# zijieli-Jlee/Temporal-Pointcloud-Upsampling-GAN

Measured on AMD Instinct MI355X. Metric: GAN train-steps/sec (G+D) on 4096-pt x3-frame clips, higher is better.
Workload: dtype bf16; 1 GPU; cfg2: 4096-pt x3-frame fluid clips, full G+D adversarial step (SRNet(3,128) + FluidTempoDis(3) + FluidSpatialDis, Adam), all-keep mask regime, gate open, even iteration; batch 8 per GPU; per_gpu_batch=8, global_batch=8, parallelism=dp1, step_mode=hipgraph (1 graph per step)

## Files before the change

### include/tpgan_ops.h

```cpp
#ifndef TPGAN_OPS_H
#define TPGAN_OPS_H

#include <stddef.h>
#include <stdint.h>

#ifdef __cplusplus
extern "C" {
#endif

typedef enum {
    TPG_OK = 0,
    TPG_ERR_ARG = -1,
    TPG_ERR_LAUNCH = -2,
    TPG_ERR_UNSUPPORTED = -3
} tpg_status;

#define TPG_MAX_K 64

const char *tpg_version(void);
const char *tpg_target_arch(void);

int tpg_knn_f32(const float *p1, const float *p2, const int64_t *len1,
                const int64_t *len2, int B, int P1, int P2, int D, int K,
                float r2, float *dist, int64_t *idx, void *stream);

int tpg_knn_grid_f32(const float *p1, const float *p2, const int64_t *len1, const int64_t *len2, int B,
                     int P1, int P2, int K, float *dist, int64_t *idx, void *ws, void *stream);

int tpg_knn_mfma_f32(const float *p1, const float *p2, const int64_t *len1,
                     const int64_t *len2, int B, int P1, int P2, int D, int K,
                     float *dist, int64_t *idx, int redo, void *stream);

int tpg_knn_small_f32(const float *p1, const float *p2, const int64_t *len1,
                      const int64_t *len2, int B, int P1, int P2, int D, int K,
                      float *dist, int64_t *idx, int redo, void *stream);

size_t tpg_frnn_grid_workspace_bytes(int B, int P2);
int tpg_frnn_grid_f32(const float *p1, const float *p2, const int64_t *len1, const int64_t *len2, int B, int P1,
                      int P2, int K, float r, float *dist, int64_t *idx, void *ws, void *stream);

int tpg_chamfer_fwd_f32(const float *src, const float *tgt, int B, int N, int M,
                        float *d1, int64_t *i1, float *d2, int64_t *i2,
                        void *stream);
size_t tpg_chamfer_bwd_workspace_bytes(int B, int N, int M);
int tpg_chamfer_bwd_f32(const float *src, const float *tgt, int B, int N, int M,
                        const int64_t *i1, const int64_t *i2, const float *g1,
                        const float *g2, float *gsrc, float *gtgt, void *ws, void *stream);

int tpg_fps_f32(const float *xyz, int B, int N, int m, float *temp, int32_t *idx,
                void *stream);

int tpg_fps_prefix_f32(const float *xyz, int B, int N, int m, float *temp, int32_t *idx,
                       const int32_t *prefix_in, int32_t *prefix_out, void *stream);

int tpg_fps_start_f32(const float *xyz, const int32_t *start, int skip_origin, int B, int N, int m,
                      float *temp, int32_t *idx, void *stream);

int tpg_gather_fwd_f32(const float *feat, const int32_t *idx, int B, int C, int N,
                       int S, float *out, void *stream);
int tpg_gather_bwd_f32(const float *gout, const int32_t *idx, int B, int C, int N,
                       int S, float *gfeat, void *stream);

int tpg_gather_rows_fwd_f32(const float *rows, const int32_t *idx, int B, int N, int S, int C, float *out, void *stream);
int tpg_gather_rows_bwd_f32(const float *gout, const int32_t *idx, int B, int N, int S, int C, float *grows,
                            void *stream);

int tpg_ball_query_f32(const float *xyz, const float *new_xyz, int B, int N, int S,
                       float radius, int nsample, int32_t *idx, void *stream);

int tpg_group_fwd_f32(const float *feat, const int32_t *idx, int B, int C, int N,
                      int S, int K, float *out, void *stream);
int tpg_group_bwd_f32(const float *gout, const int32_t *idx, int B, int C, int N,
                      int S, int K, float *gfeat, void *stream);

int tpg_three_nn_f32(const float *unknown, const float *known, int B, int n, int m,
                     float *dist2, int32_t *idx, void *stream);
int tpg_three_interp_fwd_f32(const float *feat, const int32_t *idx, const float *w,
                             int B, int C, int m, int n, float *out, void *stream);
int tpg_three_interp_bwd_f32(const float *gout, const int32_t *idx, const float *w,
                             int B, int C, int m, int n, float *gfeat,
                             void *stream);

typedef enum { TPG_DTYPE_F32 = 0, TPG_DTYPE_BF16 = 1 } tpg_dtype;

int tpg_rowcombine_fwd(const void *U, const void *QE, const int32_t *idx, int mode, int dtype_in,
                       int dtype_out, int B, int N, int S, int K, int C, float slope, void *out,
                       void *stream);

int tpg_invert_index(const int32_t *idx, int B, int N, int SK, int32_t *offs, int32_t *list,
                     int32_t *tmp, void *stream);

int tpg_rowcombine_bwd(const void *gout, const int32_t *idx, const int32_t *offs, const int32_t *list,
                       const void *E, int mode, int dtype_in, int dtype_out, int B, int N, int S, int K,
                       int C, float slope, void *gU, void *gQE, void *stream);

int tpg_rowcombine_edge_fwd(const void *Y, const int32_t *idx, int dtype_in, int dtype_out, int B, int N, int K, int C,
                            float slope_a, float slope_e, void *out, void *stream);
int tpg_rowcombine_edge_bwd(const void *gout, const int32_t *idx, const int32_t *offs, const int32_t *list,
                            const void *Y, int dtype_in, int dtype_out, int B, int N, int K, int C, float slope_a,
                            float slope_e, void *gY, void *stream);

int tpg_head_bn_act_fwd(const float *h, int B, int C, const float *gamma, const float *beta, float *running_mean,
                        float *running_var, long long *num_batches_tracked, float momentum, float eps, float slope,
                        const float *mask, float *y, float *mean, float *rstd, void *stream);
int tpg_head_bn_act_bwd(const float *gy, const float *h, const float *mean, const float *rstd, const float *gamma,
                        const float *beta, float slope, const float *mask, int B, int C, float *dh, float *dgamma,
                        float *dbeta, void *stream);

#define TPG_BN_PHASE_ALL 0
#define TPG_BN_PHASE_STATS 1
#define TPG_BN_PHASE_APPLY 2
size_t tpg_rowbn_workspace_bytes(int C, int nseg);
int tpg_rowbn_fwd(const void *x, int dtype_in, long long P, int K, int C, float eps, float momentum,
                  int training, float *running_mean, float *running_var, long long *num_batches_tracked,
                  const float *mean_shift, const float *gamma, const float *beta, float slope, float *mean,
                  float *rstd, void *y,
                  int dtype_out, uint8_t *argmax, void *ws, int nseg, int phase, void *stream);
int tpg_rowbn_bwd(const void *gy, int dtype_g, const void *x, int dtype_in, const uint8_t *argmax,
                  const void *y, int dtype_y, long long P, int K, int C, int training, const float *mean,
                  const float *rstd, const float *gamma, const float *beta, float slope, float *dgamma,
                  float *dbeta, void *dx, void *ws, int nseg, int phase, void *stream);

int tpg_rowbn_bwd_sums(const void *gy, int dtype_g, const void *x, int dtype_in, const uint8_t *argmax,
                       const void *y, int dtype_y, long long P, int K, int C, int training, const float *mean,
                       const float *rstd, const float *gamma, const float *beta, float slope, float *dgamma,
                       float *dbeta, float *c12, void *ws, int nseg, void *stream);

int tpg_rowbn_stats_consts(const void *x, int dtype_in, long long P, int C, float eps, float momentum,
                           float *running_mean, float *running_var, long long *num_batches_tracked,
                           const float *mean_shift, const float *gamma, const float *beta, float *mean, float *rstd,
                           float *ci, void *ws, int nseg, void *stream);
int tpg_rowbn_bwd_sums_consts(const void *gy, int dtype_g, const void *x, int dtype_in, const uint8_t *argmax,
                              const void *y, int dtype_y, long long P, int K, int C, int training, const float *mean,
                              const float *rstd, const float *gamma, const float *beta, float slope, float *dgamma,
                              float *dbeta, float *c12, float *cb, void *ag, void *ws, int nseg, void *stream);

size_t tpg_mlp_workspace_bytes(int C, int nseg);
int tpg_mlp_fwd(const void *x, long long P, int Cin, int Cout, int nseg, const float *ss_in, int ss_stride,
                float slope_in, const float *W, int w_per_seg, void *y, float eps, float momentum,
                float *running_mean, float *running_var, long long *num_batches_tracked, const float *mean_shift,
                const float *gamma_out, const float *beta_out, float *mean_out, float *rstd_out, float *ci_out,
                void *ws, void *stream);

int tpg_mlp_consts(const float *mean, const float *rstd, const float *gamma, const float *beta, const float *c12,
                   int C, int nseg, float *ci, float *cb, void *stream);
int tpg_mlp_max_prep(const void *gout, const void *y, const float *cb_out, float slope_out, long long rows, int C,
                     int nseg, void *ag, void *stream);
int tpg_mlp_dgrad(const void *x_out, const void *g_out, const uint8_t *arg, int K, const float *cb_out,
                  const void *x_in, const float *ci_in, float slope_in, const float *W,
                  int w_per_seg, long long P, int Cin, int Cout, int nseg, int mode, void *g_in, float *c12_in,
                  float *dgamma_in, float *dbeta_in, float *cb_in, void *ws, void *stream);
size_t tpg_mlp_wgrad_workspace_bytes(long long P, int Cin, int Cout, int nseg);
int tpg_mlp_wgrad(const void *x_out, const void *g_out, const uint8_t *arg, int K, const float *cb_out,
                  const void *x_in, const float *ci_in, float slope_in, long long P, int Cin,
                  int Cout, int nseg, int mode, float *dW, void *ws, void *stream);
int tpg_mlp_bn_bwd_apply(const void *g, const void *x, const float *ci, const float *c12, long long P, int C,
                         int nseg, void *dx, void *stream);
int tpg_mlp_bn_bwd_apply_rowsum(const void *g, const void *x, const float *ci, const float *c12, long long P, int K,
                                int C, int nseg, void *dx, float *qneg, void *stream);

int tpg_mlp_infer_supported(int C0, int C1, int C2, int K);
int tpg_mlp_infer_fwd(const void *U, const void *Q, const int32_t *idx, int dtype_in, int B, int N, int S, int K, int C0,
                      int C1, int C2, const void *W1p, const void *W2p, const float *a1, const float *c1, const float *a2,
                      const float *c2, float slope0, float slope1, float slope2, void *out, void *stream);

int tpg_spectral_norm_fwd(const float *W, float *u, float *v, int R, int Cn, int iterate, float eps,
                          float *Wsn, float *sigma, void *stream);
int tpg_spectral_norm_bwd(const float *G, const float *Wsn, const float *u, const float *v,
                          const float *sigma, int R, int Cn, float *dW, void *stream);

long long tpg_spectral_norm_multi_stride(int R, int Cn);
int tpg_spectral_norm_multi_fwd(const void *desc, int M, int max_rc, float *out, int iterate, float eps,
                                void *stream);
// ... 129 lines not shown
```

### temporal-pointcloud-upsampling-gan_amd/_lib.py

```python
import ctypes as C
import os

_HERE = os.path.dirname(os.path.abspath(__file__))
LIB_PATH = os.environ.get("TPGAN_HIP_LIBRARY") or os.path.join(_HERE, "csrc", "libtpgan_hip.so")

_P = C.c_void_p
_I = C.c_int
_F = C.c_float
_L = C.c_longlong

SIGNATURES = {
    "tpg_knn_f32": [_P, _P, _P, _P, _I, _I, _I, _I, _I, _F, _P, _P, _P],
    "tpg_knn_mfma_f32": [_P, _P, _P, _P, _I, _I, _I, _I, _I, _P, _P, _I, _P],
    "tpg_knn_small_f32": [_P, _P, _P, _P, _I, _I, _I, _I, _I, _P, _P, _I, _P],
    "tpg_knn_grid_f32": [_P, _P, _P, _P, _I, _I, _I, _I, _P, _P, _P, _P],
    "tpg_frnn_grid_f32": [_P, _P, _P, _P, _I, _I, _I, _I, _F, _P, _P, _P, _P],
    "tpg_chamfer_fwd_f32": [_P, _P, _I, _I, _I, _P, _P, _P, _P, _P],
    "tpg_chamfer_bwd_f32": [_P, _P, _I, _I, _I, _P, _P, _P, _P, _P, _P, _P, _P],
    "tpg_fps_f32": [_P, _I, _I, _I, _P, _P, _P],
    "tpg_fps_prefix_f32": [_P, _I, _I, _I, _P, _P, _P, _P, _P],
    "tpg_fps_start_f32": [_P, _P, _I, _I, _I, _I, _P, _P, _P],
    "tpg_gather_fwd_f32": [_P, _P, _I, _I, _I, _I, _P, _P],
    "tpg_gather_bwd_f32": [_P, _P, _I, _I, _I, _I, _P, _P],
    "tpg_ball_query_f32": [_P, _P, _I, _I, _I, _F, _I, _P, _P],
    "tpg_group_fwd_f32": [_P, _P, _I, _I, _I, _I, _I, _P, _P],
    "tpg_group_bwd_f32": [_P, _P, _I, _I, _I, _I, _I, _P, _P],
    "tpg_three_nn_f32": [_P, _P, _I, _I, _I, _P, _P, _P],
    "tpg_three_interp_fwd_f32": [_P, _P, _P, _I, _I, _I, _I, _P, _P],
    "tpg_three_interp_bwd_f32": [_P, _P, _P, _I, _I, _I, _I, _P, _P],
    "tpg_gather_rows_fwd_f32": [_P, _P, _I, _I, _I, _I, _P, _P],
    "tpg_gather_rows_bwd_f32": [_P, _P, _I, _I, _I, _I, _P, _P],
    "tpg_rowcombine_fwd": [_P, _P, _P, _I, _I, _I, _I, _I, _I, _I, _I, _F, _P, _P],
    "tpg_invert_index": [_P, _I, _I, _I, _P, _P, _P, _P],
    "tpg_rowcombine_bwd": [_P, _P, _P, _P, _P, _I, _I, _I, _I, _I, _I, _I, _I, _F, _P, _P, _P],
    "tpg_rowcombine_edge_fwd": [_P, _P, _I, _I, _I, _I, _I, _I, _F, _F, _P, _P],
    "tpg_rowcombine_edge_bwd": [_P, _P, _P, _P, _P, _I, _I, _I, _I, _I, _I, _F, _F, _P, _P],
    "tpg_head_bn_act_fwd": [_P, _I, _I, _P, _P, _P, _P, _P, _F, _F, _F, _P, _P, _P, _P, _P],
    "tpg_head_bn_act_bwd": [_P, _P, _P, _P, _P, _P, _F, _P, _I, _I, _P, _P, _P, _P],
    "tpg_rowbn_fwd": [_P, _I, _L, _I, _I, _F, _F, _I, _P, _P, _P, _P, _P, _P, _F, _P, _P, _P, _I, _P, _P, _I, _I, _P],
    "tpg_rowbn_bwd": [_P, _I, _P, _I, _P, _P, _I, _L, _I, _I, _I, _P, _P, _P, _P, _F, _P, _P, _P, _P, _I, _I, _P],
    "tpg_cubic_interp_f32": [_P, _P, _P, _I, _I, _I, _I, _F, _P, _P, _P, _P],
    "tpg_spectral_norm_fwd": [_P, _P, _P, _I, _I, _I, _F, _P, _P, _P],
    "tpg_spectral_norm_bwd": [_P, _P, _P, _P, _P, _I, _I, _P, _P],
    "tpg_spectral_norm_multi_fwd": [_P, _I, _I, _P, _I, _F, _P],
    "tpg_spectral_norm_multi_fwd_split": [_P, _P, _I, _I, _P, _P, _L, _F, _P],
    "tpg_spectral_norm_multi_bwd": [_P, _I, _I, _P, _P, _P, _P, _P],
    "tpg_rowbn_bwd_sums": [_P, _I, _P, _I, _P, _P, _I, _L, _I, _I, _I, _P, _P, _P, _P, _F, _P, _P, _P, _P, _I, _P],
    "tpg_rowbn_bwd_sums_consts": [_P, _I, _P, _I, _P, _P, _I, _L, _I, _I, _I, _P, _P, _P, _P, _F, _P, _P, _P, _P, _P, _P, _I, _P],
    "tpg_rowbn_stats_consts": [_P, _I, _L, _I, _F, _F, _P, _P, _P, _P, _P, _P, _P, _P, _P, _P, _I, _P],
    "tpg_mlp_consts": [_P, _P, _P, _P, _P, _I, _I, _P, _P, _P],
    "tpg_mlp_max_prep": [_P, _P, _P, _F, _L, _I, _I, _P, _P],
    "tpg_mlp_dgrad": [_P, _P, _P, _I, _P, _P, _P, _F, _P, _I, _L, _I, _I, _I, _I, _P, _P, _P, _P, _P, _P, _P],
    "tpg_mlp_wgrad": [_P, _P, _P, _I, _P, _P, _P, _F, _L, _I, _I, _I, _I, _P, _P, _P],
    "tpg_mlp_bn_bwd_apply": [_P, _P, _P, _P, _L, _I, _I, _P, _P],
    "tpg_mlp_bn_bwd_apply_rowsum": [_P, _P, _P, _P, _L, _I, _I, _I, _P, _P, _P],
    "tpg_small_tail_fwd": [_P, _I, _P, _P, _F, _F, _L, _I, _I, _I, _I, _P, _P, _P],
    "tpg_small_tail_bwd": [_P, _P, _P, _P, _I, _P, _P, _F, _F, _L, _I, _I, _I, _I, _P, _P, _P, _P, _P],
    "tpg_rowlinear_fwd": [_P, _I, _P, _P, _L, _I, _I, _I, _F, _P, _I, _P],
    "tpg_rowlinear_dgrad": [_P, _P, _I, _P, _L, _I, _I, _I, _F, _P, _I, _P],
    "tpg_rowlinear_wgrad": [_P, _I, _P, _P, _I, _L, _I, _I, _I, _F, _P, _P, _P, _P],
    "tpg_mlp_fwd": [_P, _L, _I, _I, _I, _P, _I, _F, _P, _I, _P, _F, _F, _P, _P, _P, _P, _P, _P, _P, _P, _P, _P, _P],
    "tpg_mlp_infer_fwd": [_P, _P, _P, _I, _I, _I, _I, _I, _I, _I, _I, _P, _P, _P, _P, _P, _P, _F, _F, _F, _P, _P],
    "tpg_context_expand_f32": [_P, _P, _P, _I, _I, _I, _I, _P, _P, _P, _P, _P],
    "tpg_radius_reduce_f32": [_P, _P, _P, _P, _I, _I, _I, _F, _I, _P, _P, _P, _P],
    "tpg_radius_reduce_exhaustive_f32": [_P, _P, _P, _P, _I, _I, _I, _F, _I, _P, _P, _P],
    "tpg_patch_select_f32": [_P, _L, _P, _P, _P, _I, _I, _P, _P, _P],
    "tpg_clip_gather_high_f32": [_P, _P, _L, _P, _P, _P, _I, _P, _P, _I, _I, _I, _P, _P, _P],
    "tpg_clip_gather_low_f32": [_P, _P, _P, _F, _P, _L, _P, _P, _I, _I, _I, _I, _P, _P, _P],
    "tpg_frame_subset": [_P, _P, _I, _I, _P, _P],
    "tpg_action_gather_f32": [_P, _L, _P, _P, _P, _P, _I, _I, _I, _I, _P, _P, _P],
    "tpg_replace_dummy_centres": [_P, _P, _P, _I, _I, _I, _I, _P, _P, _P, _P],
    "tpg_emd_init_f32": [_P, _I, _I, _I, _I, _P, _P, _P],
    "tpg_emd_rounds_f32": [_P, _I, _I, _F, _F, _I, _I, _I, _I, _I, _P, _P, _P],
    "tpg_emd_finish_f32": [_P, _I, _I, _P, _P, _P, _P, _P, _P],
    "tpg_gaussian_row_sums_f32": [_P, _P, _P, _P, _I, _I, _I, _F, _P, _P],
    "tpg_render_points_f32": [_P, _P, _P, _I, _I, _P, _I, _I, _I, _I, _F, _F, _P, _P, _P, _P, _P, _P],
    "tpg_render_spheres_f32": [_P, _P, _I, _I, _P, _I, _I, _I, _F, _P, _P, _P, _P],
    "tpg_surface_smooth_f32": [_P, _I, _I, _I, _I, _F, _P, _P],
    "tpg_surface_shade_f32": [_P, _P, _P, _I, _I, _P, _I, _I, _I, _F, _F, _P, _P, _P, _P, _P],
    "tpg_pbf_predict_f32": [_P, _P, _P, _P, _I, _I, _F, _F, _P, _P, _P, _P],
    "tpg_pbf_grid_f32": [_P, _P, _I, _I, _F, _P, _P],
    "tpg_pbf_lambda_f32": [_P, _P, _I, _I, _F, _F, _F, _P, _P, _P, _P],
    "tpg_pbf_dp_f32": [_P, _P, _P, _P, _I, _I, _F, _F, _F, _F, _F, _P, _P, _P, _P],
    "tpg_pbf_finish_f32": [_P, _P, _P, _I, _I, _F, _F, _F, _P, _P, _P, _P],
    "tpg_iso_count_f32": [_P, _I, _I, _I, _F, _P, _P, _P],
    "tpg_iso_emit_f32": [_P, _I, _I, _I, _P, _F, _F, _P, _L, _L, _P, _P, _P, _P],
    "tpg_aniso_kernels_f32": [_P, _P, _I, _I, _F, _F, _F, _F, _F, _F, _F, _I, _I, _P, _P, _P, _P, _P, _P],
    "tpg_aniso_kernels_exhaustive_f32": [_P, _P, _I, _I, _F, _F, _F, _F, _F, _F, _F, _I, _I, _P, _P, _P, _P, _P, _P],
    "tpg_aniso_field_f32": [_P, _P, _P, _P, _P, _P, _I, _I, _I, _F, _F, _P, _P, _P],
    "tpg_aniso_field_exhaustive_f32": [_P, _P, _P, _P, _P, _P, _I, _I, _I, _F, _F, _P, _P],
}
SIZE_GETTERS = ("tpg_rowbn_workspace_bytes", "tpg_mlp_workspace_bytes", "tpg_context_expand_workspace_bytes",
                "tpg_emd_workspace_bytes", "tpg_pbf_workspace_bytes", "tpg_iso_workspace_bytes",
                "tpg_aniso_workspace_bytes")
OTHER_GETTERS = ("tpg_spectral_norm_multi_stride", "tpg_spectral_norm_multi_bwd_scratch",
                 "tpg_mlp_wgrad_workspace_bytes", "tpg_frnn_grid_workspace_bytes", "tpg_small_tail_workspace_bytes",
                 "tpg_chamfer_bwd_workspace_bytes", "tpg_rowlinear_wgrad_workspace_bytes", "tpg_rowlinear_supported",
                 "tpg_spectral_norm_split_rows", "tpg_spectral_norm_split_max_cn", "tpg_spectral_norm_split_max_rows",
                 "tpg_patch_select_workspace_bytes", "tpg_patch_select_max_k", "tpg_mlp_infer_supported")
STRING_GETTERS = ("tpg_version", "tpg_target_arch")

STATUS = {0: "TPG_OK", -1: "TPG_ERR_ARG", -2: "TPG_ERR_LAUNCH", -3: "TPG_ERR_UNSUPPORTED"}

_lib = None


class HipLibraryMissing(RuntimeError):
    pass


def load():
    global _lib
    if _lib is not None:
        return _lib
    if not os.path.exists(LIB_PATH):
        raise HipLibraryMissing(
# ... 45 lines not shown
```

### temporal-pointcloud-upsampling-gan_amd/csrc/invert_index.hpp

```cpp
#pragma once
#include "tpg_common.hpp"

namespace tpg_inv {

constexpr int kWaves = 16;
constexpr int kThreads = kWaves * 64;
constexpr int kMaxBins = 256;
constexpr int kHist = kMaxBins * kWaves;
constexpr int kUnroll = 8;
constexpr int kMaxLdsBytes = 160 * 1024;
constexpr int kFixedInts = 2 * kHist + 64;
constexpr int kMaxCntRows = kMaxLdsBytes / 4 - kFixedInts;

struct Plan {
    int bits, passes, ebits, pack, use_cnt;
    size_t smem;
};

inline int ceil_log2(long long v) {
    int b = 0;
    while ((1LL << b) < v) ++b;
    return b;
}

// ... 109 lines not shown
    }

    for (int p = 0; p < passes; ++p) {
        volatile int *cur = hist0 + (p & 1) * kHist, *nxt = hist0 + ((p + 1) & 1) * kHist;
        const bool last = p + 1 == passes;
        const int32_t *src = p == 0 ? nullptr : (((passes - p) & 1) ? tp : ls);
        int32_t *dst = ((passes - 1 - p) & 1) ? tp : ls;
        const bool packed_in = src != nullptr && pack;
        block_exclusive_scan(cur, L, wsum, tid);
        if (!last) {
            for (int i = tid; i < L; i += kThreads) nxt[i] = 0;
            __syncthreads();
        }
        const int dshift = p ? (p - 1) * bits : 0;
        int raw[kUnroll], rawn[kUnroll];
#pragma unroll
        for (int u = 0; u < kUnroll; ++u) {
            const int i = e_lo + u * 64 + lane;
            raw[u] = i < e_hi ? (src ? src[i] : i) : 0;
        }
        for (int base = e_lo; base < e_hi; base += 64 * kUnroll) {
            int ev[kUnroll], dg[kUnroll], kh[kUnroll];
#pragma unroll
            for (int u = 0; u < kUnroll; ++u) {
                const int i = base + 64 * kUnroll + u * 64 + lane;
                rawn[u] = i < e_hi ? (src ? src[i] : i) : 0;
            }
#pragma unroll
            for (int u = 0; u < kUnroll; ++u) {
                const bool ok = base + u * 64 + lane < e_hi;
                if (packed_in) {
                    ev[u] = (int)((unsigned)raw[u] & emask);
                    kh[u] = (int)((unsigned)raw[u] >> ebits);
                    dg[u] = (kh[u] >> dshift) & dmask;
                } else {
                    ev[u] = raw[u];
                    const int dest = ok ? dest_of(id, ev[u], N) : 0;
                    kh[u] = dest >> bits;
                    dg[u] = p == 0 ? (dest & dmask) : ((kh[u] >> dshift) & dmask);
                }
            }
#pragma unroll
            for (int u = 0; u < kUnroll; ++u) {
                if (base + u * 64 >= e_hi) break;
                const bool valid = base + u * 64 + lane < e_hi;
                const int digit = dg[u];
                tpg_u64 m = __ballot(valid);
                for (int bt = 0; bt < bits; ++bt) {
                    const bool on = (digit >> bt) & 1;
                    const tpg_u64 bb = __ballot(valid && on);
                    m &= on ? bb : ~bb;
                }
                if (valid) {
                    const int rank = __popcll(m & lt), group = __popcll(m);
                    const int slot = digit * kWaves + wave;
                    const int pos = cur[slot] + rank;
                    if (last) {
                        dst[pos] = ev[u];
                    } else {
                        dst[pos] = pack ? (int)(((unsigned)kh[u] << ebits) | (unsigned)ev[u]) : ev[u];
                        const int nd = (kh[u] >> (p * bits)) & dmask;
                        atomicAdd((int *)&nxt[nd * kWaves + pos / chunk], 1);
                    }
                    if (rank == group - 1) cur[slot] = pos + 1;
                }
            }
#pragma unroll
            for (int u = 0; u < kUnroll; ++u) raw[u] = rawn[u];
        }
        __syncthreads();
    }

    if (!use_cnt) {
        for (int q = tid; q < SK; q += kThreads) {
            const int k = dest_of(id, ls[q], N);
            const int kp = q ? dest_of(id, ls[q - 1], N) : -1;
            for (int n = kp + 1; n <= k; ++n) of[n] = q;
            if (q == SK - 1)
                for (int n = k + 1; n <= N; ++n) of[n] = SK;
        }
    }
}

template <typename IdxT>
inline int launch(const IdxT *idx, int B, int N, int SK, int32_t *offs, int32_t *list, int32_t *tmp, hipStream_t st) {
    const Plan p = plan(N, SK);
    if (p.passes > 1 && !tmp) return TPG_ERR_ARG;
    if (!tpg_allow_dynamic_lds<&invert_index_kernel<IdxT>>(kMaxLdsBytes)) return TPG_ERR_UNSUPPORTED;
    hipLaunchKernelGGL((invert_index_kernel<IdxT>), dim3(B), dim3(kThreads), p.smem, st, idx, N, SK, p.bits, p.passes,
                       p.ebits, p.pack, p.use_cnt, offs, list, tmp);
    return TPG_OK;
}

}
```

### temporal-pointcloud-upsampling-gan_amd/csrc/rowgather.hip

```cpp
#include <cstdlib>

#include "invert_index.hpp"
#include "tpg_rows.hpp"

namespace {

enum { MODE_GATHER = 0, MODE_SUB = 1, MODE_EDGE = 2 };

#ifndef TPG_RC_NT_STORE
#define TPG_RC_NT_STORE 0
#endif

#ifndef TPG_RC_FWD_U
#define TPG_RC_FWD_U 1
#endif
#ifndef TPG_RC_FWD_CAP
#define TPG_RC_FWD_CAP 16384
#endif
#ifndef TPG_RC_BWD_CAP
#define TPG_RC_BWD_CAP 4096
#endif
#ifndef TPG_RC_BWD_WAVE_CAP
#define TPG_RC_BWD_WAVE_CAP 16384
#endif
// ... 321 lines not shown
        hipLaunchKernelGGL((rowcombine_fwd_kernel<TI, TO, MODE_SUB>), g, blk, 0, st, u, q, idx, N, S, K, C, slope, o, total, xo, ld, slope_u);
    else
        hipLaunchKernelGGL((rowcombine_fwd_kernel<TI, TO, MODE_EDGE>), g, blk, 0, st, u, q, idx, N, S, K, C, slope, o, total, xo, ld, slope_u);
    return TPG_OK;
}

template <typename TI, typename TG>
int bwd_go(const void *gout, const int32_t *idx, const int32_t *offs, const int32_t *list, const void *E,
           int mode, int B, int N, int S, int K, int C, float slope, void *gU, void *gQE, hipStream_t st, int ld,
           const void *Uraw, float slope_u) {
    constexpr int NE = tpg_elems<TI, TG>::NE;
    if (C % NE) return TPG_ERR_UNSUPPORTED;
    const unsigned long long total64 = (unsigned long long)B * N * (C / NE);
    const unsigned long long totq64 = (unsigned long long)B * S * (C / NE);
    if (total64 >= 0x7fffffffULL || totq64 >= 0x7fffffffULL) return TPG_ERR_ARG;
    const unsigned total = (unsigned)total64;
    const dim3 g(grid_for(total, 1u, TPG_RC_BWD_CAP)), blk(256);
    const TG *go = static_cast<const TG *>(gout);
    const TI *e = static_cast<const TI *>(E);
    TI *gu = static_cast<TI *>(gU), *gq = static_cast<TI *>(gQE);
    const TI *ur = static_cast<const TI *>(Uraw);
    const unsigned cpr = (unsigned)(C / NE);
#ifndef TPG_RC_BWD_THREAD_PER_ROW
    const bool by_wave = cpr <= 32 && (64u % cpr) == 0 && !(mode == MODE_EDGE && cpr <= 2);
#else
    const bool by_wave = false;
#endif
    const unsigned rows = (unsigned)((unsigned long long)B * N);
    const unsigned wgs = (rows + 3u) / 4u;
    const dim3 gw(wgs > TPG_RC_BWD_WAVE_CAP ? TPG_RC_BWD_WAVE_CAP : wgs);
    if (mode == MODE_EDGE) {
        if (by_wave)
            hipLaunchKernelGGL((rowcombine_bwd_wave_kernel<TI, TG, MODE_EDGE>), gw, blk, 0, st, go, idx, offs, list, e, N, S, K, C, slope, gu, gq, rows, ld, ur, slope_u);
        else
            hipLaunchKernelGGL((rowcombine_bwd_kernel<TI, TG, MODE_EDGE>), g, blk, 0, st, go, idx, offs, list, e, N, S, K, C, slope, gu, gq, total, ld, ur, slope_u);
    } else {
        if (by_wave)
            hipLaunchKernelGGL((rowcombine_bwd_wave_kernel<TI, TG, MODE_GATHER>), gw, blk, 0, st, go, idx, offs, list, e, N, S, K, C, slope, gu, gq, rows, ld, ur, slope_u);
        else
            hipLaunchKernelGGL((rowcombine_bwd_kernel<TI, TG, MODE_GATHER>), g, blk, 0, st, go, idx, offs, list, e, N, S, K, C, slope, gu, gq, total, ld, ur, slope_u);
        if (mode == MODE_SUB) {
            const unsigned totq = (unsigned)totq64;
            hipLaunchKernelGGL((rowsum_neg_kernel<TI, TG>), dim3(grid_for(totq)), blk, 0, st, go, K, C, gq, totq);
        }
    }
    return TPG_OK;
}

#define TPG_DISPATCH2(din, dout, CALL)                                                   \
    ((din) == TPG_DTYPE_F32 ? ((dout) == TPG_DTYPE_F32 ? CALL(float, float) : CALL(float, __hip_bfloat16)) \
                            : ((dout) == TPG_DTYPE_F32 ? CALL(__hip_bfloat16, float)                    \
                                                       : CALL(__hip_bfloat16, __hip_bfloat16)))

}

extern "C" int tpg_rowcombine_fwd(const void *U, const void *QE, const int32_t *idx, int mode, int dtype_in,
                                  int dtype_out, int B, int N, int S, int K, int C, float slope, void *out,
                                  void *stream) {
    if (B < 0 || N <= 0 || S < 0 || K < 0 || C <= 0 || mode < 0 || mode > 2) return TPG_ERR_ARG;
    if ((long long)B * S * K == 0) return TPG_OK;
    if (!U || !idx || !out || (mode != MODE_GATHER && !QE)) return TPG_ERR_ARG;
    if (mode == MODE_EDGE && S != N) return TPG_ERR_ARG;
    if (!dtype_ok(dtype_in) || !dtype_ok(dtype_out) || !aligned16(U, QE, out, nullptr)) return TPG_ERR_UNSUPPORTED;
    hipStream_t st = tpg_stream(stream);
#define TPG_FWD(TI, TO) fwd_go<TI, TO>(U, QE, idx, mode, B, N, S, K, C, slope, out, st, C, 1.0f)
    const int rc = TPG_DISPATCH2(dtype_in, dtype_out, TPG_FWD);
#undef TPG_FWD
    if (rc) return rc;
    TPG_RETURN_IF_LAUNCH_FAILED();
    return TPG_OK;
}

extern "C" int tpg_invert_index(const int32_t *idx, int B, int N, int SK, int32_t *offs, int32_t *list,
                                int32_t *tmp, void *stream) {
    if (B < 0 || N <= 0 || SK < 0) return TPG_ERR_ARG;
    if (B == 0) return TPG_OK;
    if (!idx || !offs || !list) return TPG_ERR_ARG;
    const int rc = tpg_inv::launch<int32_t>(idx, B, N, SK, offs, list, tmp, tpg_stream(stream));
    if (rc) return rc;
    TPG_RETURN_IF_LAUNCH_FAILED();
    return TPG_OK;
}

extern "C" int tpg_rowcombine_bwd(const void *gout, const int32_t *idx, const int32_t *offs,
                                  const int32_t *list, const void *E, int mode, int dtype_in, int dtype_out,
                                  int B, int N, int S, int K, int C, float slope, void *gU, void *gQE,
                                  void *stream) {
    if (B < 0 || N <= 0 || S < 0 || K < 0 || C <= 0 || mode < 0 || mode > 2) return TPG_ERR_ARG;
    if (B == 0) return TPG_OK;
    if (!gout || !idx || !offs || !list || !gU) return TPG_ERR_ARG;
    if (mode == MODE_EDGE && (S != N || !E || !gQE)) return TPG_ERR_ARG;
    if (mode == MODE_SUB && !gQE) return TPG_ERR_ARG;
    if (!dtype_ok(dtype_in) || !dtype_ok(dtype_out) || !aligned16(gout, gU, gQE, E)) return TPG_ERR_UNSUPPORTED;
    hipStream_t st = tpg_stream(stream);
#define TPG_BWD(TI, TG) bwd_go<TI, TG>(gout, idx, offs, list, E, mode, B, N, S, K, C, slope, gU, gQE, st, C, nullptr, 1.0f)
    const int rc = TPG_DISPATCH2(dtype_in, dtype_out, TPG_BWD);
#undef TPG_BWD
    if (rc) return rc;
    TPG_RETURN_IF_LAUNCH_FAILED();
    return TPG_OK;
}

extern "C" int tpg_rowcombine_edge_fwd(const void *Y, const int32_t *idx, int dtype_in, int dtype_out, int B, int N,
                                       int K, int C, float slope_a, float slope_e, void *out, void *stream) {
    if (B < 0 || N <= 0 || K < 0 || C <= 0) return TPG_ERR_ARG;
    if ((long long)B * N * K == 0) return TPG_OK;
    if (!Y || !idx || !out) return TPG_ERR_ARG;
    if (!dtype_ok(dtype_in) || !dtype_ok(dtype_out) || !aligned16(Y, out, nullptr, nullptr)) return TPG_ERR_UNSUPPORTED;
    const int esz = dtype_in == TPG_DTYPE_F32 ? 4 : 2;
    if (((size_t)C * esz) & 15) return TPG_ERR_UNSUPPORTED;
    const char *y = static_cast<const char *>(Y);
    const void *A = y + (size_t)C * esz, *E = y;
    hipStream_t st = tpg_stream(stream);
#define TPG_FWD(TI, TO) fwd_go<TI, TO>(A, E, idx, MODE_EDGE, B, N, N, K, C, slope_e, out, st, 2 * C, slope_a)
    const int rc = TPG_DISPATCH2(dtype_in, dtype_out, TPG_FWD);
#undef TPG_FWD
    if (rc) return rc;
    TPG_RETURN_IF_LAUNCH_FAILED();
    return TPG_OK;
}

extern "C" int tpg_rowcombine_edge_bwd(const void *gout, const int32_t *idx, const int32_t *offs, const int32_t *list,
                                       const void *Y, int dtype_in, int dtype_out, int B, int N, int K, int C,
                                       float slope_a, float slope_e, void *gY, void *stream) {
    if (B < 0 || N <= 0 || K < 0 || C <= 0) return TPG_ERR_ARG;
    if (B == 0) return TPG_OK;
    if (!gout || !idx || !offs || !list || !Y || !gY) return TPG_ERR_ARG;
    if (!dtype_ok(dtype_in) || !dtype_ok(dtype_out) || !aligned16(gout, gY, Y, nullptr)) return TPG_ERR_UNSUPPORTED;
    const int esz = dtype_in == TPG_DTYPE_F32 ? 4 : 2;
    if (((size_t)C * esz) & 15) return TPG_ERR_UNSUPPORTED;
    const char *y = static_cast<const char *>(Y);
    char *gy = static_cast<char *>(gY);
    const void *A = y + (size_t)C * esz, *E = y;
    void *gA = gy + (size_t)C * esz, *gE = gy;
    hipStream_t st = tpg_stream(stream);
#define TPG_BWD(TI, TG) bwd_go<TI, TG>(gout, idx, offs, list, E, MODE_EDGE, B, N, N, K, C, slope_e, gA, gE, st, 2 * C, A, slope_a)
    const int rc = TPG_DISPATCH2(dtype_in, dtype_out, TPG_BWD);
#undef TPG_BWD
    if (rc) return rc;
    TPG_RETURN_IF_LAUNCH_FAILED();
    return TPG_OK;
}
```

### temporal-pointcloud-upsampling-gan_amd/ops.py

```python
import ctypes as C

import os

import numpy as np
import torch

from . import _lib

_BACKENDS = {}


class OpTimer:

    def __init__(self):
        self.pending = {}

    def record(self, name, nbytes, stream_of, launch, flops=0):
        st = torch.cuda.current_stream(stream_of.device)
        a = torch.cuda.Event(enable_timing=True)
        b = torch.cuda.Event(enable_timing=True)
        a.record(st)
        out = launch()
        b.record(st)
        self.pending.setdefault(name, []).append((a, b, nbytes, flops))
# ... 512 lines not shown
        return g

    def gather_rows_fwd(self, rows, idx):
        B, N, Cc = rows.shape
        S = idx.shape[1]
        out = torch.empty((B, S, Cc), dtype=torch.float32, device=rows.device)
        self._call("tpg_gather_rows_fwd_f32", "gather_fwd", 4 * B * S * (2 * Cc + 1), rows,
                   _ptr(rows), _ptr(idx), B, N, S, Cc, _ptr(out))
        return out

    def gather_rows_bwd(self, gout, idx, N):
        B, S, Cc = gout.shape
        g = torch.empty((B, N, Cc), dtype=torch.float32, device=gout.device)
        self._call("tpg_gather_rows_bwd_f32", "gather_bwd", 4 * B * (Cc * N + S + 2 * Cc * S), gout,
                   _ptr(gout), _ptr(idx), B, N, S, Cc, _ptr(g))
        return g

    def ball_query(self, radius, nsample, xyz, new_xyz):
        B, N, _ = xyz.shape
        S = new_xyz.shape[1]
        idx = torch.empty((B, S, nsample), dtype=torch.int32, device=xyz.device)
        self._call("tpg_ball_query_f32", "ball_query", 12 * B * (N + S) + 4 * B * S * nsample, xyz,
                   _ptr(xyz), _ptr(new_xyz), B, N, S, float(radius), nsample, _ptr(idx))
        return idx

    def group_fwd(self, feat, idx):
        B, Cc, N = feat.shape
        _, S, K = idx.shape
        out = torch.empty((B, Cc, S, K), dtype=torch.float32, device=feat.device)
        self._call("tpg_group_fwd_f32", "group_fwd", 4 * B * (Cc * N + S * K + Cc * S * K), feat,
                   _ptr(feat), _ptr(idx), B, Cc, N, S, K, _ptr(out))
        return out

    def group_bwd(self, gout, idx, N):
        B, Cc, S, K = gout.shape
        g = torch.empty((B, Cc, N), dtype=torch.float32, device=gout.device)
        self._call("tpg_group_bwd_f32", "group_bwd", 4 * B * (Cc * N + S * K + Cc * S * K), gout,
                   _ptr(gout), _ptr(idx), B, Cc, N, S, K, _ptr(g))
        return g

    def three_nn(self, unknown, known):
        B, n, _ = unknown.shape
        m = known.shape[1]
        d2 = torch.empty((B, n, 3), dtype=torch.float32, device=unknown.device)
        idx = torch.empty((B, n, 3), dtype=torch.int32, device=unknown.device)
        self._call("tpg_three_nn_f32", "three_nn", 12 * B * (n + m) + 24 * B * n, unknown,
                   _ptr(unknown), _ptr(known), B, n, m, _ptr(d2), _ptr(idx))
        return d2, idx

    def three_interp_fwd(self, feat, idx, w):
        B, Cc, m = feat.shape
        n = idx.shape[1]
        out = torch.empty((B, Cc, n), dtype=torch.float32, device=feat.device)
        self._call("tpg_three_interp_fwd_f32", "three_interp_fwd", 4 * B * (Cc * m + 6 * n + Cc * n), feat,
                   _ptr(feat), _ptr(idx), _ptr(w), B, Cc, m, n, _ptr(out))
        return out

    def three_interp_bwd(self, gout, idx, w, m):
        B, Cc, n = gout.shape
        g = torch.empty((B, Cc, m), dtype=torch.float32, device=gout.device)
        self._call("tpg_three_interp_bwd_f32", "three_interp_bwd", 4 * B * (Cc * m + 6 * n + Cc * n), gout,
                   _ptr(gout), _ptr(idx), _ptr(w), B, Cc, m, n, _ptr(g))
        return g

    def rowcombine_fwd(self, U, QE, idx, mode, slope, out_dtype):
        B, N, Cc = U.shape
        _, S, K = idx.shape
        out = torch.empty((B, S, K, Cc), dtype=out_dtype, device=U.device)
        nbytes = (U.element_size() * B * Cc * (N + (S if QE is not None else 0)) + 4 * B * S * K
                  + out.element_size() * B * S * K * Cc)
        self._call("tpg_rowcombine_fwd", "rowcombine_fwd", nbytes, U,
                   _ptr(U), _ptr(QE), _ptr(idx), mode, _DTYPE_CODE[U.dtype], _DTYPE_CODE[out_dtype],
                   B, N, S, K, Cc, float(slope), _ptr(out))
        return out

    def invert_index(self, idx, N):
        B = idx.shape[0]
        SK = idx[0].numel()
        offs = torch.empty((B, N + 1), dtype=torch.int32, device=idx.device)
        lst = torch.empty((B, SK), dtype=torch.int32, device=idx.device)
        tmp = torch.empty((B, SK), dtype=torch.int32, device=idx.device) if N > 256 else None
        self._call("tpg_invert_index", "invert_index", 4 * B * (2 * SK + N + 1), idx,
                   _ptr(idx), B, N, SK, _ptr(offs), _ptr(lst), _ptr(tmp))
        return offs, lst

    def rowcombine_bwd(self, gout, idx, E, mode, N, slope, in_dtype, inverse=None):
        B, S, K, Cc = gout.shape
        if inverse is None:
            inverse = self.invert_index(idx, N)
        offs, lst = inverse
        gU = torch.empty((B, N, Cc), dtype=in_dtype, device=gout.device)
        gQE = torch.empty((B, S, Cc), dtype=in_dtype, device=gout.device) if mode != 0 else None
        nbytes = (gout.element_size() * B * S * K * Cc * (2 if mode == 1 else 1) + 8 * B * S * K
                  + gU.element_size() * B * Cc * (N + (S if mode else 0)))
        self._call("tpg_rowcombine_bwd", "rowcombine_bwd", nbytes, gout,
                   _ptr(gout), _ptr(idx), _ptr(offs), _ptr(lst), _ptr(E), mode, _DTYPE_CODE[in_dtype],
                   _DTYPE_CODE[gout.dtype], B, N, S, K, Cc, float(slope), _ptr(gU), _ptr(gQE))
        return gU, gQE


    def rowcombine_edge_fwd(self, Y, idx, slope_a, slope_e, out_dtype):
        B, N, C2 = Y.shape
        Cc, K = C2 // 2, idx.shape[2]
        out = torch.empty((B, N, K, Cc), dtype=out_dtype, device=Y.device)
        nbytes = Y.element_size() * B * N * C2 + 4 * B * N * K + out.element_size() * B * N * K * Cc
        self._call("tpg_rowcombine_edge_fwd", "rowcombine_fwd", nbytes, Y,
                   _ptr(Y), _ptr(idx), _DTYPE_CODE[Y.dtype], _DTYPE_CODE[out_dtype], B, N, K, Cc, float(slope_a),
                   float(slope_e), _ptr(out))
        return out

    def rowcombine_edge_bwd(self, gout, idx, Y, slope_a, slope_e, inverse=None):
        B, N, K, Cc = gout.shape
        if inverse is None:
            inverse = self.invert_index(idx, N)
        offs, lst = inverse
        gY = torch.empty_like(Y)
        nbytes = gout.element_size() * B * N * K * Cc * 2 + 8 * B * N * K + 2 * Y.element_size() * B * N * 2 * Cc
        self._call("tpg_rowcombine_edge_bwd", "rowcombine_bwd", nbytes, gout,
                   _ptr(gout), _ptr(idx), _ptr(offs), _ptr(lst), _ptr(Y), _DTYPE_CODE[Y.dtype], _DTYPE_CODE[gout.dtype],
                   B, N, K, Cc, float(slope_a), float(slope_e), _ptr(gY))
        return gY

    def head_bn_act_fwd(self, h, gamma, beta, running_mean, running_var, nbt, momentum, eps, slope, mask):
        B, Cc = h.shape
        y = torch.empty_like(h)
        mean = torch.empty(Cc, dtype=torch.float32, device=h.device)
        rstd = torch.empty(Cc, dtype=torch.float32, device=h.device)
        self._call("tpg_head_bn_act_fwd", "head_bn_act", 4 * B * Cc * (3 if mask is not None else 2), h,
                   _ptr(h), B, Cc, _ptr(gamma), _ptr(beta), _ptr(running_mean), _ptr(running_var), _ptr(nbt),
                   float(momentum), float(eps), float(slope), _ptr(mask), _ptr(y), _ptr(mean), _ptr(rstd))
        return y, mean, rstd

    def head_bn_act_bwd(self, gy, h, mean, rstd, gamma, beta, slope, mask, need_affine):
        B, Cc = h.shape
        dh = torch.empty_like(h)
        dg = torch.empty(Cc, dtype=torch.float32, device=h.device) if need_affine else None
        db = torch.empty(Cc, dtype=torch.float32, device=h.device) if need_affine else None
        self._call("tpg_head_bn_act_bwd", "head_bn_act_bwd", 4 * B * Cc * (4 if mask is not None else 3), h,
                   _ptr(gy), _ptr(h), _ptr(mean), _ptr(rstd), _ptr(gamma), _ptr(beta), float(slope), _ptr(mask), B, Cc,
                   _ptr(dh), _ptr(dg), _ptr(db))
        return dh, dg, db

    def _bn_ws(self, x, C_, nseg=1):
        need = self.lib.tpg_rowbn_workspace_bytes(max(C_, 256), max(nseg, 1)) // 4
        return self._workspace("rowbn", x, need, zeroed=True)

    def rowbn_fwd(self, x, K, eps, momentum, training, running_mean, running_var, gamma, beta, slope,
                  mean, rstd, out_dtype, num_batches_tracked=None, nseg=1, mean_shift=None):
        P, Cc = x.shape
        rows = P // K if K else P
        y = torch.empty((rows, Cc), dtype=out_dtype, device=x.device)
        arg = torch.empty((rows, Cc), dtype=torch.uint8, device=x.device) if K else None
        ws = self._bn_ws(x, Cc, nseg)
        args = (_ptr(x), _DTYPE_CODE[x.dtype], P, K, Cc, float(eps), float(momentum), int(training),
                _ptr(running_mean), _ptr(running_var), _ptr(num_batches_tracked), _ptr(mean_shift), _ptr(gamma),
                _ptr(beta),
                float(slope), _ptr(mean),
                _ptr(rstd), _ptr(y), _DTYPE_CODE[out_dtype], _ptr(arg), _ptr(ws), int(nseg))
        b_stats = x.element_size() * P * Cc
        b_apply = x.element_size() * P * Cc + y.element_size() * rows * Cc + (rows * Cc if K else 0)
        if _timer is None:
            self._call("tpg_rowbn_fwd", "rowbn_fwd", b_stats + b_apply, x, *args, 0)
        else:
            if training:
                self._call("tpg_rowbn_fwd", "rowbn_fwd_stats", b_stats, x, *args, 1)
            self._call("tpg_rowbn_fwd", "rowbn_fwd_apply_max" if K else "rowbn_fwd_apply", b_apply, x, *args, 2)
# ... 2300 lines not shown
```

Before: 83.42 steps/s.

## Split index inversion across destination slices with multiple workgroups per batch

Adds a sliced invert-index kernel in which each workgroup owns a contiguous range of destination rows. It counts per-wave entries in LDS, scans them, and ranks entries through a per-wave ring with ballot-based stable ranking. This replaces the single-workgroup-per-batch two-pass radix sort when N and SK fit the heuristics, so many more CUs are used and the tmp buffer pass is avoided. The cost is that every workgroup rescans the whole index array, so the total reads of idx grow with the number of slices.

```diff
diff --git a/include/tpgan_ops.h b/include/tpgan_ops.h
--- a/include/tpgan_ops.h
+++ b/include/tpgan_ops.h
@@ -89,6 +89,11 @@
 
 int tpg_invert_index(const int32_t *idx, int B, int N, int SK, int32_t *offs, int32_t *list,
                      int32_t *tmp, void *stream);
+
+int tpg_invert_index_sliced(const int32_t *idx, int B, int N, int SK, int slice_dests, int32_t *offs,
+                            int32_t *list, void *stream);
+int tpg_invert_index_slice_dests(int B, int N, int SK);
+int tpg_invert_index_sliced_const(int which);
 
 int tpg_rowcombine_bwd(const void *gout, const int32_t *idx, const int32_t *offs, const int32_t *list,
                        const void *E, int mode, int dtype_in, int dtype_out, int B, int N, int S, int K,
diff --git a/temporal-pointcloud-upsampling-gan_amd/_lib.py b/temporal-pointcloud-upsampling-gan_amd/_lib.py
--- a/temporal-pointcloud-upsampling-gan_amd/_lib.py
+++ b/temporal-pointcloud-upsampling-gan_amd/_lib.py
@@ -32,6 +32,9 @@
     "tpg_gather_rows_bwd_f32": [_P, _P, _I, _I, _I, _I, _P, _P],
     "tpg_rowcombine_fwd": [_P, _P, _P, _I, _I, _I, _I, _I, _I, _I, _I, _F, _P, _P],
     "tpg_invert_index": [_P, _I, _I, _I, _P, _P, _P, _P],
+    "tpg_invert_index_sliced": [_P, _I, _I, _I, _I, _P, _P, _P],
+    "tpg_invert_index_slice_dests": [_I, _I, _I],
+    "tpg_invert_index_sliced_const": [_I],
     "tpg_rowcombine_bwd": [_P, _P, _P, _P, _P, _I, _I, _I, _I, _I, _I, _I, _I, _F, _P, _P, _P],
     "tpg_rowcombine_edge_fwd": [_P, _P, _I, _I, _I, _I, _I, _I, _F, _F, _P, _P],
     "tpg_rowcombine_edge_bwd": [_P, _P, _P, _P, _P, _I, _I, _I, _I, _I, _I, _F, _F, _P, _P],
diff --git a/temporal-pointcloud-upsampling-gan_amd/csrc/invert_index.hpp b/temporal-pointcloud-upsampling-gan_amd/csrc/invert_index.hpp
--- a/temporal-pointcloud-upsampling-gan_amd/csrc/invert_index.hpp
+++ b/temporal-pointcloud-upsampling-gan_amd/csrc/invert_index.hpp
@@ -215,10 +215,175 @@
     }
 }
 
+constexpr int kRing = 128;
+constexpr int kSlicedFixedInts = 64 + kWaves * 2 * kRing;
+
+inline size_t sliced_smem(int D) { return sizeof(int) * ((size_t)D * kWaves + kSlicedFixedInts); }
+
+template <typename IdxT, typename F>
+__device__ __forceinline__ void for_each_step(const IdxT *id, int e_lo, int e_hi, int N, int lane, F &&f) {
+    int d[kUnroll], dn[kUnroll];
+#pragma unroll
+    for (int u = 0; u < kUnroll; ++u) {
+        const int i = e_lo + u * 64 + lane;
+        d[u] = i < e_hi ? dest_of(id, i, N) : -1;
+    }
+    for (int base = e_lo; base < e_hi; base += 64 * kUnroll) {
+#pragma unroll
+        for (int u = 0; u < kUnroll; ++u) {
+            const int i = base + 64 * kUnroll + u * 64 + lane;
+            dn[u] = i < e_hi ? dest_of(id, i, N) : -1;
+        }
+#pragma unroll
+        for (int u = 0; u < kUnroll; ++u) {
+            if (base + u * 64 >= e_hi) break;
+            f(base + u * 64 + lane, d[u]);
+        }
+#pragma unroll
+        for (int u = 0; u < kUnroll; ++u) d[u] = dn[u];
+    }
+}
+
+template <typename IdxT>
+__global__ __launch_bounds__(kThreads) void invert_index_sliced_kernel(const IdxT *__restrict__ idx, int B, int N, int SK,
+                                                                       int D, int G, int xcd_order,
+                                                                       int32_t *__restrict__ offs,
+                                                                       int32_t *__restrict__ list) {
+    extern __shared__ __attribute__((aligned(16))) int inv_smem[];
+    const int tid = threadIdx.x, lane = tid & 63, wave = tid >> 6;
+    const unsigned lb = xcd_order ? (blockIdx.x & 7u) * (gridDim.x >> 3) + (blockIdx.x >> 3) : blockIdx.x;
+    if (lb >= (unsigned)B * (unsigned)G) return;
+    const int b = (int)(lb / (unsigned)G), g = (int)(lb % (unsigned)G);
+    const int lo = g * D, hi = min(lo + D, N), Dl = hi - lo;
+    volatile int *cnt = inv_smem;
+    volatile int *wsum = inv_smem + Dl * kWaves;
+    volatile int *re = wsum + 64 + wave * 2 * kRing, *rd = re + kRing;
+    const IdxT *id = idx + (size_t)b * SK;
+    int32_t *of = offs + (size_t)b * (N + 1);
+    int32_t *ls = list + (size_t)b * SK;
+    const int L = Dl * kWaves;
+    const int bits = Dl > 1 ? 32 - __clz(Dl - 1) : 0;
+    const int chunk = (((SK + kWaves - 1) / kWaves) + 63) & ~63;
+    const int e_lo = min(wave * chunk, SK), e_hi = min(e_lo + chunk, SK);
+    const tpg_u64 lt = lane ? (~0ULL >> (64 - lane)) : 0ULL;
+
+    for (int i = tid; i < L; i += kThreads) cnt[i] = 0;
+    __syncthreads();
+    int below = 0;
+    for_each_step(id, e_lo, e_hi, N, lane, [&](int, int d) {
+        if (d >= 0) {
+            const int r = d - lo;
+            if ((unsigned)r < (unsigned)Dl) atomicAdd((int *)&cnt[r * kWaves + wave], 1);
+            below += r < 0;
+        }
+    });
+#pragma unroll
+    for (int o = 32; o; o >>= 1) below += __shfl_xor(below, o);
+    if (lane == 0) wsum[32 + wave] = below;
+    __syncthreads();
+    int base = 0;
+#pragma unroll
+    for (int w = 0; w < kWaves; ++w) base += wsum[32 + w];
+
+    block_exclusive_scan(cnt, L, wsum, tid);
+    for (int r = tid; r < Dl; r += kThreads) of[lo + r] = base + cnt[r * kWaves];
+    if (g == G - 1 && tid == 0) of[N] = SK;
+    __syncthreads();
+
+    int fill = 0, head = 0;
+    auto rank_batch = [&](int n) {
+        const bool valid = lane < n;
+        const int q = (head + lane) & (kRing - 1);
+        const int e = valid ? re[q] : 0, r = valid ? rd[q] : 0;
+        tpg_u64 m = __ballot(valid);
+        for (int bt = 0; bt < bits; ++bt) {
+            const bool on = (r >> bt) & 1;
+            const tpg_u64 bb = __ballot(valid && on);
+            m &= on ? bb : ~bb;
+        }
+        if (valid) {
+            const int rank = __popcll(m & lt), group = __popcll(m);
+            const int slot = r * kWaves + wave;
+            const int pos = cnt[slot] + rank;
+            ls[base + pos] = e;
+            if (rank == group - 1) cnt[slot] = pos + 1;
+        }
+        head += n;
+    };
+    for_each_step(id, e_lo, e_hi, N, lane, [&](int e, int d) {
+        const int r = d - lo;
+        const bool in = d >= 0 && (unsigned)r < (unsigned)Dl;
+        const tpg_u64 m = __ballot(in);
+        if (m == 0) return;
+        if (in) {
+            const int q = (fill + __popcll(m & lt)) & (kRing - 1);
+            re[q] = e;
+            rd[q] = r;
+        }
+        fill += __popcll(m);
+        if (fill - head >= 64) rank_batch(64);
+    });
+    if (fill > head) rank_batch(fill - head);
+}
+
+#ifndef TPG_INV_SLICE_MIN_DESTS
+#define TPG_INV_SLICE_MIN_DESTS 256
+#endif
+#ifndef TPG_INV_SLICE_WIDEST_DESTS
+#define TPG_INV_SLICE_WIDEST_DESTS 1024
+#endif
+#ifndef TPG_INV_SLICE_MAX_DESTS
+#define TPG_INV_SLICE_MAX_DESTS 2048
+#endif
+#ifndef TPG_INV_SLICED_MIN_DESTS
+#define TPG_INV_SLICED_MIN_DESTS 512
+#endif
+#ifndef TPG_INV_SLICED_MIN_ENTRIES
+#define TPG_INV_SLICED_MIN_ENTRIES 2048
+#endif
+#ifndef TPG_INV_SLICED_MIN_FILL
+#define TPG_INV_SLICED_MIN_FILL 4
+#endif
+#ifndef TPG_INV_SLICED_MAX_WGS
+#define TPG_INV_SLICED_MAX_WGS 256
+#endif
+static_assert(TPG_INV_SLICE_MAX_DESTS * kWaves + kSlicedFixedInts <= kMaxLdsBytes / 4, "a slice's counters fit the LDS");
+
+inline int sliced_dests_for(int B, int N, int SK) {
+    const Plan p = plan(N, SK);
+    if (B <= 0 || p.passes != 2 || !p.use_cnt || N < TPG_INV_SLICED_MIN_DESTS || SK < TPG_INV_SLICED_MIN_ENTRIES ||
+        SK < (long long)TPG_INV_SLICED_MIN_FILL * N)
+        return 0;
+    for (int D = TPG_INV_SLICE_MIN_DESTS; D <= TPG_INV_SLICE_WIDEST_DESTS; D *= 2) {
+        const long long G = (N + D - 1) / D;
+        if (G < 2) return 0;
+        if ((long long)B * G <= TPG_INV_SLICED_MAX_WGS) return D;
+    }
+    return 0;
+}
+
+template <typename IdxT>
+inline int launch_sliced(const IdxT *idx, int B, int N, int SK, int D, int32_t *offs, int32_t *list, hipStream_t st) {
+    if (D < 1 || D > TPG_INV_SLICE_MAX_DESTS) return TPG_ERR_UNSUPPORTED;
+    if (D > N) D = N;
+    const long long G = (N + D - 1) / D, wgs = (long long)B * G;
+    if (wgs + 7 >= 0x7fffffffLL) return TPG_ERR_UNSUPPORTED;
+    if (!tpg_allow_dynamic_lds<&invert_index_sliced_kernel<IdxT>>(kMaxLdsBytes)) return TPG_ERR_UNSUPPORTED;
+    static const bool xcd_on = [] { const char *e = getenv("TPG_RC_XCD"); return !(e && e[0] == '0'); }();
+    const int xo = xcd_on && wgs >= 16;
+    const unsigned nb = xo ? (unsigned)((wgs + 7) & ~7LL) : (unsigned)wgs;
+    hipLaunchKernelGGL((invert_index_sliced_kernel<IdxT>), dim3(nb), dim3(kThreads), sliced_smem(D), st, idx, B, N, SK, D,
+                       (int)G, xo, offs, list);
+    return TPG_OK;
+}
+
 template <typename IdxT>
 inline int launch(const IdxT *idx, int B, int N, int SK, int32_t *offs, int32_t *list, int32_t *tmp, hipStream_t st) {
     const Plan p = plan(N, SK);
     if (p.passes > 1 && !tmp) return TPG_ERR_ARG;
+    static const bool sliced_on = [] { const char *e = getenv("TPG_INV_SLICED"); return !(e && e[0] == '0'); }();
+    const int D = sliced_on ? sliced_dests_for(B, N, SK) : 0;
+    if (D) return launch_sliced<IdxT>(idx, B, N, SK, D, offs, list, st);
     if (!tpg_allow_dynamic_lds<&invert_index_kernel<IdxT>>(kMaxLdsBytes)) return TPG_ERR_UNSUPPORTED;
     hipLaunchKernelGGL((invert_index_kernel<IdxT>), dim3(B), dim3(kThreads), p.smem, st, idx, N, SK, p.bits, p.passes,
                        p.ebits, p.pack, p.use_cnt, offs, list, tmp);
diff --git a/temporal-pointcloud-upsampling-gan_amd/csrc/rowgather.hip b/temporal-pointcloud-upsampling-gan_amd/csrc/rowgather.hip
--- a/temporal-pointcloud-upsampling-gan_amd/csrc/rowgather.hip
+++ b/temporal-pointcloud-upsampling-gan_amd/csrc/rowgather.hip
@@ -427,6 +427,32 @@
     return TPG_OK;
 }
 
+extern "C" int tpg_invert_index_sliced(const int32_t *idx, int B, int N, int SK, int slice_dests, int32_t *offs,
+                                       int32_t *list, void *stream) {
+    if (B < 0 || N <= 0 || SK < 0) return TPG_ERR_ARG;
+    if (B == 0) return TPG_OK;
+    if (!idx || !offs || !list) return TPG_ERR_ARG;
+    const int rc = tpg_inv::launch_sliced<int32_t>(idx, B, N, SK, slice_dests, offs, list, tpg_stream(stream));
+    if (rc) return rc;
+    TPG_RETURN_IF_LAUNCH_FAILED();
+    return TPG_OK;
+}
+
+extern "C" int tpg_invert_index_slice_dests(int B, int N, int SK) { return tpg_inv::sliced_dests_for(B, N, SK); }
+
+extern "C" int tpg_invert_index_sliced_const(int which) {
+    switch (which) {
+        case 0: return TPG_INV_SLICE_MIN_DESTS;
+        case 1: return TPG_INV_SLICE_WIDEST_DESTS;
+        case 2: return TPG_INV_SLICED_MIN_DESTS;
+        case 3: return TPG_INV_SLICED_MIN_ENTRIES;
+        case 4: return TPG_INV_SLICED_MAX_WGS;
+        case 5: return TPG_INV_SLICE_MAX_DESTS;
+        case 6: return TPG_INV_SLICED_MIN_FILL;
+        default: return -1;
+    }
+}
+
 extern "C" int tpg_rowcombine_bwd(const void *gout, const int32_t *idx, const int32_t *offs,
                                   const int32_t *list, const void *E, int mode, int dtype_in, int dtype_out,
                                   int B, int N, int S, int K, int C, float slope, void *gU, void *gQE,
diff --git a/temporal-pointcloud-upsampling-gan_amd/ops.py b/temporal-pointcloud-upsampling-gan_amd/ops.py
--- a/temporal-pointcloud-upsampling-gan_amd/ops.py
+++ b/temporal-pointcloud-upsampling-gan_amd/ops.py
@@ -618,6 +618,15 @@
         tmp = torch.empty((B, SK), dtype=torch.int32, device=idx.device) if N > 256 else None
         self._call("tpg_invert_index", "invert_index", 4 * B * (2 * SK + N + 1), idx,
                    _ptr(idx), B, N, SK, _ptr(offs), _ptr(lst), _ptr(tmp))
+        return offs, lst
+
+    def invert_index_sliced(self, idx, N, slice_dests):
+        B = idx.shape[0]
+        SK = idx[0].numel()
+        offs = torch.empty((B, N + 1), dtype=torch.int32, device=idx.device)
+        lst = torch.empty((B, SK), dtype=torch.int32, device=idx.device)
+        self._call("tpg_invert_index_sliced", "invert_index", 4 * B * (2 * SK + N + 1), idx,
+                   _ptr(idx), B, N, SK, int(slice_dests), _ptr(offs), _ptr(lst))
         return offs, lst
 
     def rowcombine_bwd(self, gout, idx, E, mode, N, slope, in_dtype, inverse=None):
```

Result: no change. 83.18 steps/s (-0.3%).
